# arkworks-rs/circom-compat

Hardware: AMD Instinct MI355X
Metric: Groth16 constraints/sec (BN254) (higher is better)
Workload: dtype int32x9 (29-bit limbs of 254-bit Montgomery integers); 1 GPU; synthetic squaring-chain R1CS, 2^22-2 constraints, BN254, full prove (witness map + 4 G1 MSM + 1 G2 MSM + finalize), trapdoor key minted on GPU; log2_domain=22, num_constraints=4194302, n_vars=4194304, parallelism=single-gpu

## Files before the change

circom_compat_amd/csrc/api.hip:

```cpp
#include "../../include/g16_amd.h"

#include <stddef.h>
#include <stdlib.h>

#include <algorithm>
#include <mutex>

#include "ctx.h"

using namespace g16;

static_assert(offsetof(g16::ProofSums, B1) == sizeof(g16::G1XYZZ29) && offsetof(g16::ProofSums, L) == 2 * sizeof(g16::G1XYZZ29),
              "ProofSums must keep A, B1, L adjacent (batched reduction writes them as an array)");
static_assert(G16_PARTIAL_BYTES == g16::FIN_PARTIAL_BYTES, "partial record size out of sync");

namespace {
std::mutex g_err_mu;
std::string g_create_error;
}


namespace {

g16_status fail(g16_ctx* ctx, g16_status code, const std::string& msg) {
  if (ctx) ctx->err = msg;
  else {
    std::lock_guard<std::mutex> g(g_err_mu);
    g_create_error = msg;
  }
  return code;
}

template <class Fn>
g16_status guarded(g16_ctx* ctx, Fn fn) {
  try {
    if (ctx) G16_HIP(hipSetDevice(ctx->device));
    return fn();
  } catch (const HipError& e) {
    return fail(ctx, G16_ERR_HIP, e.what());
  } catch (const std::bad_alloc&) {
    return fail(ctx, G16_ERR_INTERNAL, "host allocation failed");
  } catch (const std::exception& e) {
    const bool dom = std::string(e.what()).find("PolynomialDegreeTooLarge") != std::string::npos;
    return fail(ctx, dom ? G16_ERR_DOMAIN_TOO_LARGE : G16_ERR_INTERNAL, e.what());
  }
}

void shard(uint32_t len, int rank, int world, uint32_t* lo, uint32_t* hi) {
  *lo = (uint32_t)((uint64_t)len * rank / world);
  *hi = (uint32_t)((uint64_t)len * (rank + 1) / world);
}

int work1_batch(const MsmConfig& cw, uint32_t wr, bool sharded) {
  return (cw.nb() / wr < (1u << 18) || sharded) ? 3 : 2;
}

size_t msm_state_bytes(const MsmConfig& cw, const MsmConfig& ch, uint32_t lw, uint32_t l_cnt, uint32_t lh,
                       uint32_t wr, bool sharded, bool own_w, bool own_h, bool view_w) {
  size_t b = 0;
  if (view_w) b += MsmSort::view_bytes_for(lw, cw);
  if (own_w) b += (size_t)cw.Pn * ((size_t)lw * (64 * 2 + 128) + (size_t)l_cnt * 64);
  if (own_h) b += (size_t)ch.Pn * lh * 64;
  b += MsmSort::bytes_for(lw, cw) + MsmSort::bytes_for(lh, ch);
  const uint32_t nc_w = ceil_div(cw.B, msm_red_chunk(cw, 1, wr)) * cw.D;
  const uint32_t nc_h = ceil_div(ch.B, msm_red_chunk(ch)) * ch.D;
  const uint32_t slots_w = cw.nb() + cw.max_lanes(), slots_h = ch.nb() + ch.max_lanes();
  b += msm_work_bytes<Fq>(slots_w, nc_w, cw.D, work1_batch(cw, wr, sharded)) + msm_work_bytes<Fq2>(slots_w, nc_w, cw.D, 1) +
       msm_work_bytes<Fq>(slots_h, nc_h, ch.D, 1);
  return b;
}

void plan_msm_configs(const g16_options& o, uint32_t lw, uint32_t l_cnt, uint32_t lh, uint32_t wr, bool sharded,
                      bool own_w, bool own_h, bool view_w, MsmConfig* cw, MsmConfig* ch) {
  if (own_w) *cw = msm_make_config(lw ? lw : 1, o.window_bits, o.planes);
  if (own_h) *ch = msm_make_config(lh ? lh : 1, o.window_bits, o.planes);
  if (o.planes > 0) return;
  size_t fr = 0, tot = 0;
  if (hipMemGetInfo(&fr, &tot) != hipSuccess) return;
  const size_t margin = std::min(((size_t)2 << 30) + fr / 50, fr / 4);
  const size_t budget = fr - margin;
  if (msm_state_bytes(*cw, *ch, lw, l_cnt, lh, wr, sharded, own_w, own_h, view_w) <= budget) return;
  auto layouts = [&](const MsmConfig& full, uint32_t len, bool own) {
    std::vector<MsmConfig> v{full};
    for (int pn = full.Pn - 1; own && pn >= 1; --pn) {
      const MsmConfig c = msm_make_config(len ? len : 1, o.window_bits, pn);
      if (c.Pn != v.back().Pn) v.push_back(c);
    }
    return v;
  };
  const std::vector<MsmConfig> vw = layouts(*cw, lw, own_w), vh = layouts(*ch, lh, own_h);
  long best = -1;
  size_t best_bytes = 0;
  for (const MsmConfig& a : vw)
    for (const MsmConfig& b : vh) {
      const size_t need = msm_state_bytes(a, b, lw, l_cnt, lh, wr, sharded, own_w, own_h, view_w);
      if (need > budget) continue;
      const long score = 5L * a.D + b.D;
      if (best < 0 || score < best || (score == best && need > best_bytes)) {
        best = score;
        best_bytes = need;
        *cw = a;
        *ch = b;
      }
    }
  if (best < 0) {
    if (!own_w && !own_h)
      throw std::runtime_error("the sort and partial-sum state of this ctx does not fit the device memory that is free (" +
                               std::to_string(fr >> 20) + " MiB)");
    throw std::runtime_error("the proving key does not fit this device's memory even with one plane per point (" +
                             std::to_string(fr >> 20) + " MiB free)");
  }
}

inline bool sched_r5() {
  static const bool v = [] { const char* e = getenv("G16_SCHED_R5"); return e && atoi(e) != 0; }();
  return v;
}

void collect_times(g16_ctx* c) {
  if (c->timer.enabled) c->timer.collect(c->st_ms, c->st_cnt);
}

struct BucketChunk {
  uint32_t count;
  const Fr* w;
  size_t w_stride;
  int32_t *abc, *spmv;
  U256* h;
  ProofSums* sums;
  MsmSort *sort_w, *sort_h, *sort_b;
  MsmWork<Fq> *work1, *workH;
  MsmWork<Fq2>* work2;
  Fr* rs;
  const uint8_t* rs_host;
  FinScratch* scr;
  uint8_t *rec, *proj;
  uint32_t rec_stride;
  uint8_t *rec_host, *proj_host;
  const MsmSort& sort_for_b(const g16_ctx* c) const { return c->sparse_b ? *sort_b : *sort_w; }
};

BucketChunk own_chunk(g16_ctx* c, const Fr* w_dev) {
  return BucketChunk{1,           w_dev,       c->N,        c->wm.abc.p, c->wm.spmv.partial.p, c->h_canon.p, c->sums_dev.p,
                     &c->sort_w,  &c->sort_h,  &c->sort_b,  &c->work1,   &c->workH,            &c->work2,
                     c->rs_dev.p, c->pin_io,   c->fin_scr.p, c->out_dev.p, c->part_dev(), (uint32_t)G16_PROOF_BYTES,
                     c->pin_io + 64, c->pin_io + 64 + G16_PROOF_BYTES};
}

void accumulate_ab(g16_ctx* c, const BucketChunk& ch, hipStream_t s, StageTimer* tm, bool fixup = true) {
  if (c->ptsA.stride == 2) {
    msm_accumulate_pair<Fq>(*ch.sort_w, c->ptsA, c->ptsB1, *ch.work1, 0, s, tm, fixup);
  } else {
    msm_accumulate<Fq>(*ch.sort_w, c->ptsA, 0, *ch.work1, 0, s, tm, fixup);
    msm_accumulate<Fq>(*ch.sort_w, c->ptsB1, 0, *ch.work1, 1, s, tm, fixup);
  }
}
void fixup_ab(g16_ctx* c, const BucketChunk& ch, hipStream_t q) {
  StageTimer* tm = c->timer.enabled ? &c->timer : nullptr;
  if (c->ptsA.stride == 2) {
    msm_fixup_pair<Fq>(*ch.sort_w, c->ptsA, c->ptsB1, *ch.work1, 0, q, tm);
  } else {
    msm_fixup<Fq>(*ch.sort_w, c->ptsA, 0, *ch.work1, 0, q, tm);
    msm_fixup<Fq>(*ch.sort_w, c->ptsB1, 0, *ch.work1, 1, q, tm);
  }
}

void enqueue_witness_sort(g16_ctx* c, const BucketChunk& ch) {
  hipStream_t s = c->stream;
  StageTimer* tm = c->timer.enabled ? &c->timer : nullptr;
  int id = tm ? tm->begin(ST_MSM_SORT, s) : -1;
  ch.sort_w->run(ch.w + 1 + c->w_lo, c->w_hi - c->w_lo, true, s, ch.count, ch.w_stride);
  if (tm) tm->end(id, s);
  if (c->sparse_b) {
    hipStream_t v = c->overlap ? c->red : s;
    G16_HIP(hipEventRecord(c->ev_view, s));
    G16_HIP(hipStreamWaitEvent(v, c->ev_view, 0));
    id = tm ? tm->begin(ST_MSM_SORT, v) : -1;
    ch.sort_b->run_view(*ch.sort_w, c->keep_b, v);
    if (tm) tm->end(id, v);
    G16_HIP(hipEventRecord(c->ev_view, v));
  }
}
void wait_for_b_view(g16_ctx* c, hipStream_t s) {
  if (c->sparse_b) G16_HIP(hipStreamWaitEvent(s, c->ev_view, 0));
}

template <class Hook, class Hook2>
void enqueue_witness_msms(g16_ctx* c, const BucketChunk& ch, Hook after_ab, Hook2 after_b2, bool sorted = false) {
  hipStream_t s = c->stream;
  StageTimer* tm = c->timer.enabled ? &c->timer : nullptr;
  ProofSums* S = ch.sums;
  const size_t ps = sizeof(ProofSums);
  if (!sorted) enqueue_witness_sort(c, ch);
  const uint32_t nb_eff = ch.count * c->cfg_w.nb() / (c->shard_buckets ? (uint32_t)c->world : 1u);
  const bool small = nb_eff < (1u << 18);
  const uint32_t b2_limit = c->world > 1 ? (1u << 18) : (1u << 16);
  const bool b2_off = c->overlap && nb_eff < b2_limit;
  const bool sharded = c->world > 1 || c->dist_wm;
  const bool mid = (nb_eff >= (1u << 15) && small) || (sharded && nb_eff >= (1u << 15));
  if (mid && c->overlap && ch.work1->batch >= 3) {
    hipStream_t q = c->red;
    accumulate_ab(c, ch, s, tm, false);
    G16_HIP(hipEventRecord(c->ev_acc[0], s));
    G16_HIP(hipStreamWaitEvent(q, c->ev_acc[0], 0));
    fixup_ab(c, ch, q);
    msm_reduce<Fq>(*ch.sort_w, *ch.work1, 0, 2, &S->A, q, tm, true, ps);
    after_ab(q);
    wait_for_b_view(c, s);
    msm_accumulate<Fq2>(ch.sort_for_b(c), c->ptsB2, 0, *ch.work2, 0, s, tm);
    G16_HIP(hipEventRecord(c->ev_acc[1], s));
    G16_HIP(hipStreamWaitEvent(q, c->ev_acc[1], 0));
    msm_reduce<Fq2>(ch.sort_for_b(c), *ch.work2, 0, 1, &S->B2, q, tm, true, ps);
    const bool r5 = sched_r5();
    hipStream_t ql = r5 ? q : c->side;
    if (!r5) after_b2();
    msm_accumulate<Fq>(*ch.sort_w, c->ptsL, c->l_idx_min, *ch.work1, 2, s, tm, false);
    G16_HIP(hipEventRecord(c->ev_acc[2], s));
    G16_HIP(hipStreamWaitEvent(ql, c->ev_acc[2], 0));
    msm_fixup<Fq>(*ch.sort_w, c->ptsL, c->l_idx_min, *ch.work1, 2, ql, tm);
    msm_reduce<Fq>(*ch.sort_w, *ch.work1, 2, 1, &S->L, ql, tm, true, ps);
    if (r5) after_b2();
    G16_HIP(hipEventRecord(c->ev_b2, q));
    G16_HIP(hipStreamWaitEvent(c->side, c->ev_b2, 0));
    G16_HIP(hipEventRecord(c->ev_side, c->side));
    return;
  }
  if (small && ch.work1->batch >= 3) {
    accumulate_ab(c, ch, s, tm);
    msm_accumulate<Fq>(*ch.sort_w, c->ptsL, c->l_idx_min, *ch.work1, 2, s, tm);
    msm_reduce<Fq>(*ch.sort_w, *ch.work1, 0, 3, &S->A, s, tm, false, ps);
    after_ab(s);
  } else {
    accumulate_ab(c, ch, s, tm);
    msm_reduce<Fq>(*ch.sort_w, *ch.work1, 0, 2, &S->A, s, tm, false, ps);
    after_ab(s);
    msm_run<Fq>(*ch.sort_w, c->ptsL, c->l_idx_min, *ch.work1, &S->L, s, tm, ps);
  }
  wait_for_b_view(c, s);
  msm_accumulate<Fq2>(ch.sort_for_b(c), c->ptsB2, 0, *ch.work2, 0, s, tm);
  hipStream_t rs = b2_off ? c->red : s;
  G16_HIP(hipEventRecord(c->ev_b2, s));
  G16_HIP(hipStreamWaitEvent(rs, c->ev_b2, 0));
  msm_reduce<Fq2>(ch.sort_for_b(c), *ch.work2, 0, 1, &S->B2, rs, tm, false, ps);
  G16_HIP(hipEventRecord(c->ev_b2, rs));
  if (rs != c->red) G16_HIP(hipStreamWaitEvent(c->red, c->ev_b2, 0));
  after_b2();
  G16_HIP(hipEventRecord(c->ev_b2, c->red));
  G16_HIP(hipStreamWaitEvent(c->side, c->ev_b2, 0));
  G16_HIP(hipEventRecord(c->ev_side, c->side));
}

void enqueue_h_msm(g16_ctx* c, const BucketChunk& ch) {
  hipStream_t s = c->stream;
  StageTimer* tm = c->timer.enabled ? &c->timer : nullptr;
  G16_HIP(hipStreamWaitEvent(s, c->ev_h, 0));
  msm_run<Fq>(*ch.sort_h, c->ptsH, 0, *ch.workH, &ch.sums->H, s, tm, sizeof(ProofSums));
}

template <class Hook, class Hook2>
void run_msms(g16_ctx* c, const BucketChunk& ch, Hook after_ab, Hook2 after_b2) {
  hipStream_t s = c->stream, x = c->overlap ? c->aux : c->stream;
  StageTimer* tm = c->timer.enabled ? &c->timer : nullptr;
  const uint32_t nb_eff = ch.count * c->cfg_w.nb() / (c->shard_buckets ? (uint32_t)c->world : 1u);
  const bool sort_first = !sched_r5() && c->overlap && c->world == 1 && nb_eff >= (1u << 18) && c->n <= (1u << 24);
  if (sort_first) enqueue_witness_sort(c, ch);
  G16_HIP(hipEventRecord(c->ev_w, s));
  G16_HIP(hipStreamWaitEvent(x, c->ev_w, 0));
  int id = tm ? tm->begin(ST_WITNESS_MAP, x) : -1;
  c->wm.run_batch(ch.w, ch.w_stride, ch.count, ch.abc, ch.spmv, ch.h, nullptr, x);
  if (tm) tm->end(id, x);
  id = tm ? tm->begin(ST_MSM_SORT, x) : -1;
  ch.sort_h->run(ch.h + c->h_lo, c->h_hi - c->h_lo, false, x, ch.count, c->wm.n);
  if (tm) tm->end(id, x);
  G16_HIP(hipEventRecord(c->ev_h, x));
  enqueue_witness_msms(c, ch, after_ab, after_b2, sort_first);
  enqueue_h_msm(c, ch);
}

template <class Hook>
void run_msms(g16_ctx* c, const BucketChunk& ch, Hook after_ab) {
// ... 209 lines not shown

g16_status ctx_create_impl(const g16_key_desc* key, const g16_csr* a, const g16_csr* b,
                           uint32_t num_constraints, const g16_options* opt, g16_ctx* share_from,
                           g16_ctx** out, std::string* err) {
  auto bad = [&](g16_status code, const std::string& msg) {
    if (err) *err = msg;
    return code;
  };
  if (!key || !a || !b || !out) return bad(G16_ERR_INVALID, "null argument");
  *out = nullptr;
  g16_options o{};
  if (opt) o = *opt;
  if (o.world <= 0) o.world = 1;
  if (o.rank < 0 || o.rank >= o.world) return bad(G16_ERR_INVALID, "bad rank/world");
  if (o.shard < G16_SHARD_AUTO || o.shard > G16_SHARD_BUCKETS) return bad(G16_ERR_INVALID, "unknown shard mode");
  if ((uint64_t)key->n_vars < (uint64_t)key->n_public + 1)
    return bad(G16_ERR_INVALID, "n_vars < n_public+1");
  for (const g16_csr* mtx : {a, b}) {
    if (!mtx->row_ptr || (mtx->nnz && (!mtx->col || !mtx->coeff)))
      return bad(G16_ERR_INVALID, "matrix with null arrays");
    if (mtx->row_ptr[0] != 0 || mtx->row_ptr[num_constraints] != mtx->nnz)
      return bad(G16_ERR_INVALID, "matrix row_ptr does not span [0, nnz]");
    for (uint32_t i = 0; i < num_constraints; ++i)
      if (mtx->row_ptr[i] > mtx->row_ptr[i + 1])
        return bad(G16_ERR_INVALID, "matrix row_ptr is not monotone");
    for (uint64_t j = 0; j < mtx->nnz; ++j)
      if (mtx->col[j] >= key->n_vars)
        return bad(G16_ERR_INVALID, "matrix wire index >= n_vars");
  }
  int ndev = 0;
  if (hipGetDeviceCount(&ndev) != hipSuccess || ndev <= 0)
    return bad(G16_ERR_NO_DEVICE, "no HIP device visible: this library has no CPU fallback");
  if (o.device < 0 || o.device >= ndev) return bad(G16_ERR_INVALID, "bad device ordinal");
  if (share_from && (share_from->device != o.device || !share_from->has_key || share_from->multi ||
                     !(share_from->shard_buckets || (share_from->world == 1 && o.world == 1 && !share_from->dist_wm && o.dist_wm <= 0))))
    return bad(G16_ERR_INVALID, "planes can only be shared with a whole-key ctx on the same device");

  g16_ctx* c = new (std::nothrow) g16_ctx();
  if (!c) return bad(G16_ERR_INTERNAL, "host allocation failed");
  c->device = o.device;
  c->rank = o.rank;
  c->world = o.world;
  g16_status st = guarded(c, [&]() -> g16_status {
    G16_HIP(hipStreamCreateWithFlags(&c->stream, hipStreamNonBlocking));
    G16_HIP(hipStreamCreateWithFlags(&c->side, hipStreamNonBlocking));
    G16_HIP(hipStreamCreateWithFlags(&c->red, hipStreamNonBlocking));
    {
      int lo = 0, hi = 0;
      G16_HIP(hipDeviceGetStreamPriorityRange(&lo, &hi));
      (void)lo;
      G16_HIP(hipStreamCreateWithPriority(&c->aux, hipStreamNonBlocking, hi));
    }
    if (const char* e = getenv("G16_NO_OVERLAP")) c->overlap = !(e[0] == '1');
    G16_HIP(hipEventCreateWithFlags(&c->ev_w, hipEventDisableTiming));
    G16_HIP(hipEventCreateWithFlags(&c->ev_h, hipEventDisableTiming));
    G16_HIP(hipEventCreateWithFlags(&c->ev_start, hipEventDisableTiming));
    G16_HIP(hipEventCreateWithFlags(&c->ev_ab, hipEventDisableTiming));
    G16_HIP(hipEventCreateWithFlags(&c->ev_side, hipEventDisableTiming));
    G16_HIP(hipEventCreateWithFlags(&c->ev_b2, hipEventDisableTiming));
    for (auto& e : c->ev_acc) G16_HIP(hipEventCreateWithFlags(&e, hipEventDisableTiming));
    G16_HIP(hipEventCreateWithFlags(&c->ev_fixed, hipEventDisableTiming));
    G16_HIP(hipEventCreateWithFlags(&c->ev_view, hipEventDisableTiming));
    G16_HIP(hipEventCreateWithFlags(&c->ev_send, hipEventDisableTiming));
    G16_HIP(hipEventCreateWithFlags(&c->ev_part, hipEventDisableTiming));
    G16_HIP(hipEventCreateWithFlags(&c->ev_user, hipEventDisableTiming));
    hipStream_t s = c->stream;
    c->N = key->n_vars;
    c->p = key->n_public;
    c->num_inputs = c->p + 1;
    c->m = num_constraints;
    c->nnz_a = a->nnz;
    c->nnz_b = b->nnz;
    CsrHost A{a->row_ptr, a->col, (const Fr*)a->coeff, (size_t)a->nnz};
    CsrHost B{b->row_ptr, b->col, (const Fr*)b->coeff, (size_t)b->nnz};
    if (o.reduction != G16_REDUCTION_CIRCOM && o.reduction != G16_REDUCTION_LIBSNARK)
      throw std::runtime_error("unknown reduction");
    c->dist_wm = o.dist_wm > 0;
    if (c->dist_wm && o.reduction != G16_REDUCTION_CIRCOM)
      throw std::runtime_error("the distributed witness map implements CircomReduction only");
    if (c->dist_wm) {
      c->wd.init(A, B, c->m, c->num_inputs, c->rank, c->world);
      c->n = c->wd.n;
    } else {
      c->wm.init(A, B, c->m, c->num_inputs, o.reduction);
      c->n = c->wm.n;
    }
    if (key->domain_size != c->n)
      throw std::runtime_error("key domain_size does not match num_constraints + num_inputs");

    const uint32_t len_w = c->N - 1;
    c->has_key = key->a_query != nullptr;
    c->shard_buckets = c->world > 1 && c->has_key && o.shard == G16_SHARD_BUCKETS;
    c->share_from = (c->shard_buckets || c->world == 1) ? share_from : nullptr;
    if (c->share_from) ++c->share_from->borrowers;
    shard(len_w, c->rank, c->world, &c->w_lo, &c->w_hi);
    shard(c->n, c->rank, c->world, &c->h_lo, &c->h_hi);
    if (c->dist_wm) {
      c->h_lo = 0;
      c->h_hi = c->n / (uint32_t)c->world;
    }
    if (c->shard_buckets) {
      c->w_lo = 0;
      c->w_hi = len_w;
    }
    const uint32_t lw = c->w_hi - c->w_lo, lh = c->h_hi - c->h_lo;
    const uint32_t wr = c->shard_buckets ? (uint32_t)c->world : 1u;
// ... 966 lines not shown
```

circom_compat_amd/csrc/ctx.h:

```cpp
#pragma once
#include <atomic>
#include "../../include/g16_amd.h"

#include <memory>
#include <string>

#include "finalize.h"
#include "msm_table.h"
#include "msm.h"
#include "witness_map.h"
#include "wm_dist.h"

namespace g16 {
struct Multi;
}

struct g16_ctx {
  int device = 0, rank = 0, world = 1;
  uint32_t N = 0, p = 0, n = 0, m = 0, num_inputs = 0;
  bool has_key = false;
  bool overlap = true;
  hipStream_t stream = nullptr;
  hipStream_t side = nullptr;
  hipStream_t aux = nullptr;
  hipStream_t red = nullptr;
  hipEvent_t ev_start = nullptr, ev_ab = nullptr, ev_side = nullptr, ev_w = nullptr, ev_h = nullptr,
             ev_b2 = nullptr, ev_fixed = nullptr, ev_view = nullptr;
  hipEvent_t ev_acc[3] = {nullptr, nullptr, nullptr};
  hipEvent_t ev_send = nullptr;
  hipEvent_t ev_part = nullptr;
  hipEvent_t ev_user = nullptr;
  hipStream_t xstream = nullptr;
  bool have_xstream = false;
  void* nccl_comm = nullptr;
  int nccl_ranks = 0;
  hipStream_t xs_own = nullptr;
  g16::DevBuf<uint8_t> xsend, xrecv;
  std::string err;

  g16::WitnessMap wm;
  g16::WmDist wd;
  bool dist_wm = false;
  bool fixed_ready = false;
  uint64_t fixed_rs[8] = {0};
  bool shard_buckets = false;
  uint32_t w_lo = 0, w_hi = 0, h_lo = 0, h_hi = 0;
  uint32_t l_idx_min = 0;
  g16::MsmConfig cfg_w, cfg_h;
  g16::MsmSort sort_w, sort_h;
  g16::MsmSort sort_b;
  g16::DevBuf<uint32_t> keep_b_own;
  const uint32_t* keep_b = nullptr;
  bool sparse_b = false;
  uint32_t b_inf_points = 0;
  const g16::MsmSort& sort_for_b() const { return sparse_b ? sort_b : sort_w; }
  g16::MsmPoints<g16::Fq> ptsA, ptsB1, ptsL, ptsH;
  g16::MsmPoints<g16::Fq2> ptsB2;
  g16::MsmWork<g16::Fq> work1, workH;
  g16::MsmWork<g16::Fq2> work2;
  g16::TableSet tbl;

  g16::DevBuf<g16::Fr> w_dev, h_dev, rs_dev;
  g16::DevBuf<g16::U256> h_canon;
  g16::DevBuf<g16::KeyHeaderDev> key_dev;
  g16::DevBuf<g16::ProofSums> sums_dev;
  g16::DevBuf<g16::FinTables> fin_tab;
  g16::DevBuf<g16::FinScratch> fin_scr;
  g16::DevBuf<uint8_t> out_dev;
  void* pinned_w = nullptr;
  uint8_t* pin_io = nullptr;

  struct BatchWs {
    uint32_t cap = 0;
    g16::DevBuf<g16::Fr> w, rs;
// ... 58 lines not shown
```

circom_compat_amd/csrc/msm.h:

```cpp
#pragma once
#include <stdlib.h>
#include "common.h"
#include "ec29.h"

namespace g16 {

constexpr int MSM_ACC_THREADS = 128;
#ifdef G16_EMU
constexpr int MSM_ACC_BLOCKS = 48;
constexpr int MSM_ACC_BLOCKS_G2 = 32;
#else
constexpr int MSM_ACC_BLOCKS = 3072;
constexpr int MSM_ACC_BLOCKS_G2 = 2048;
#endif
constexpr int MSM_MIN_SEG = 8;
constexpr int MSM_SMALL_MULTI = 32;
constexpr int MSM_RED_CHUNK = 16;
constexpr uint32_t MSM_IDX_BITS_WIDE = 27, MSM_IDX_BITS_NARROW = 26;

struct MsmConfig {
  int c = 0;
  int W = 0;
  int Pn = 1;
  int D = 0;
// ... 92 lines not shown
  const Affine<F>* view = nullptr;
  uint32_t stride = 1, off = 0;
  const Affine<F>* data() const { return view ? view : pts.p; }
  void init(const Affine<F>* host_points, uint32_t count, const MsmConfig& cfg, hipStream_t stream);
  static void init_pair(MsmPoints& a, MsmPoints& b, const Affine<F>* host_a, const Affine<F>* host_b,
                        uint32_t count, const MsmConfig& cfg, hipStream_t stream);
  void init_from_device(const Affine<F>* dev_points, uint32_t count, const MsmConfig& cfg,
                        hipStream_t stream);
};

#ifdef G16_EMU
constexpr uint32_t MSM_FIX_CAP = 512;
#else
constexpr uint32_t MSM_FIX_CAP = 2048;
#endif
struct MsmFixList {
  uint32_t count;
  uint32_t overflow;
  uint32_t slot[MSM_FIX_CAP];
  uint32_t entry[MSM_FIX_CAP];
};

template <class F>
struct MsmWork {
  int batch = 1;
  uint32_t slots = 0, ncontrib = 0;
  int sets = 1;
  DevBuf<MsmAcc<F>> partial;
  DevBuf<MsmAcc<F>> contrib;
  DevBuf<MsmAcc<F>> bsum;
  DevBuf<MsmAcc<F>> wsum;
  DevBuf<MsmFixList> fix;
  void init(uint32_t n_slots, uint32_t n_contrib, int max_sets, int batch = 1);
};

template <class F>
inline size_t msm_work_bytes(uint32_t n_slots, uint32_t n_contrib, int max_sets, int batch) {
  return (size_t)batch * ((size_t)n_slots + n_contrib + (size_t)257 * max_sets) * sizeof(MsmAcc<F>) +
         (size_t)batch * sizeof(MsmFixList);
}

template <class F>
void msm_run(const MsmSort& s, const MsmPoints<F>& pts, uint32_t idx_min, MsmWork<F>& work,
             MsmAcc<F>* out_dev, hipStream_t stream, StageTimer* tm = nullptr, size_t out_stride = 0);
template <class F>
void msm_accumulate(const MsmSort& s, const MsmPoints<F>& pts, uint32_t idx_min, MsmWork<F>& work,
                    int slot, hipStream_t stream, StageTimer* tm = nullptr, bool fixup = true);
template <class F>
void msm_fixup(const MsmSort& s, const MsmPoints<F>& pts, uint32_t idx_min, MsmWork<F>& work, int slot,
               hipStream_t stream, StageTimer* tm = nullptr);
template <class F>
void msm_accumulate_pair(const MsmSort& s, const MsmPoints<F>& a, const MsmPoints<F>& b,
                         MsmWork<F>& work, int slot, hipStream_t stream, StageTimer* tm = nullptr,
                         bool fixup = true);
template <class F>
void msm_fixup_pair(const MsmSort& s, const MsmPoints<F>& a, const MsmPoints<F>& b, MsmWork<F>& work,
                    int slot, hipStream_t stream, StageTimer* tm = nullptr);
template <class F>
void msm_reduce(const MsmSort& s, MsmWork<F>& work, int first_slot, int nbatch, MsmAcc<F>* out_dev,
                hipStream_t stream, StageTimer* tm = nullptr, bool hidden = false, size_t out_stride = 0);
inline uint32_t msm_contrib_cap(const MsmConfig& cfg, uint32_t nproof_cap) {
  uint32_t m = 1;
  for (uint32_t z = 1; z <= nproof_cap; ++z)
    for (uint32_t nbatch = 1; nbatch <= 3; ++nbatch)
      for (int hidden = 0; hidden < 2; ++hidden) {
        const uint32_t rc = msm_red_chunk(cfg, nbatch * z, 1, hidden != 0);
        const uint32_t v = (uint32_t)(((uint64_t)cfg.B + rc - 1) / rc) * (uint32_t)cfg.D * z;
        if (v > m) m = v;
      }
  return m;
}



}
```

circom_compat_amd/csrc/msm_curve.inc.h:

```cpp
#pragma once
#include <stdlib.h>

#include "msm.h"

namespace g16 {

namespace {

constexpr int ACC_THREADS = MSM_ACC_THREADS;
constexpr uint32_t MSM_EXACT_BLOCKS = 256;

inline bool acc_fast() {
  static const bool v = [] { const char* e = getenv("G16_ACC_FAST"); return !e || atoi(e) != 0; }();
  return v;
}
template <class F>
constexpr bool acc_is_g1() { return sizeof(F) == sizeof(Fq); }
constexpr int COMB_THREADS = 64;
constexpr int SUM_THREADS = 128;

template <class F>
__global__ void __launch_bounds__(128) k_precompute_planes(Affine<F>* pts, uint32_t count, int Pn,
                                                           int shift_bits, uint32_t stride,
                                                           uint32_t off) {
  using LF = typename Lazy<F>::type;
  const uint32_t i = blockIdx.x * blockDim.x + threadIdx.x;
  if (i >= count) return;
  pts += off;
  const Aff29<LF> p0 = affine_from_mont256<F>(pts[(size_t)i * stride]);
  pts[(size_t)i * stride] = store_packed_affine<F>(p0);
  XYZZ29<LF> q = XYZZ29<LF>::from_affine(p0);
  for (int j = 1; j < Pn; ++j) {
    for (int s = 0; s < shift_bits; ++s) q.dbl_in_place();
    pts[((size_t)j * count + i) * stride] = store_packed_affine<F>(q.to_affine());
  }
}

__device__ __forceinline__ uint32_t bucket_of(const uint32_t* __restrict__ offset, uint32_t nb,
                                              uint32_t pos) {
  uint32_t lo = 0, hi = nb;
  while (hi - lo > 1) {
    const uint32_t mid = (lo + hi) >> 1;
    if (offset[mid] <= pos) lo = mid;
    else hi = mid;
  }
  return lo;
}

template <class F>
struct AccWay {
  using LF = typename Lazy<F>::type;
  uint32_t seg, pos, end, g, bend, bnext, en_next, en_next2;
  bool live;
  XYZZ29<LF> acc;
  Affine<F> raw_next;
};

__device__ uint32_t g_gather_mask = 0xffffffffu;

template <class F, int PS>
__device__ __forceinline__ void acc_fetch(const Affine<F>* __restrict__ pts, uint32_t npts,
                                          uint32_t idx_min, uint32_t idx_bits, uint32_t en,
                                          Affine<F>& raw) {
  const uint32_t idx = en & ((1u << idx_bits) - 1u);
  if (idx >= idx_min) {
    const uint32_t plane = (en & 0x7fffffffu) >> idx_bits;
#ifdef G16_DEBUG_GATHER
    raw = pts[((size_t)(plane & g_gather_mask) * npts + ((idx - idx_min) & g_gather_mask)) * PS];
#else
    raw = pts[((size_t)plane * npts + (idx - idx_min)) * PS];
#endif
  } else {
    raw = Affine<F>::infinity();
  }
}

template <class F, int PS>
__device__ __forceinline__ void acc_way_init(AccWay<F>& w, uint32_t seg, uint32_t S, uint32_t M,
                                             const Affine<F>* __restrict__ pts, uint32_t npts,
                                             uint32_t idx_min, uint32_t idx_bits,
                                             const uint32_t* __restrict__ entries,
                                             const uint32_t* __restrict__ offset, uint32_t nb) {
  w.seg = seg;
  w.pos = seg * S;
  w.live = w.pos < M;
  w.end = w.live ? (w.pos + S < M ? w.pos + S : M) : w.pos;
  w.acc = XYZZ29<typename Lazy<F>::type>::infinity();
  w.raw_next = Affine<F>::infinity();
  w.g = 0;
  w.bend = w.bnext = 0;
  w.en_next = w.en_next2 = 0;
  if (w.live) {
    w.g = bucket_of(offset, nb, w.pos);
    w.bend = offset[w.g + 1];
    w.bnext = offset[w.g + 2 < nb ? w.g + 2 : nb];
    w.en_next = entries[w.pos];
    w.en_next2 = w.pos + 1 < w.end ? entries[w.pos + 1] : 0u;
    acc_fetch<F, PS>(pts, npts, idx_min, idx_bits, w.en_next, w.raw_next);
  }
}

template <class F, int PS>
__device__ __forceinline__ Aff29<typename Lazy<F>::type> acc_way_prepare(
    AccWay<F>& w, bool* step, const Affine<F>* __restrict__ pts, uint32_t npts, uint32_t idx_min,
    uint32_t idx_bits, const uint32_t* __restrict__ entries, const uint32_t* __restrict__ offset,
    uint32_t nb, MsmAcc<F>* __restrict__ partial) {
  using LF = typename Lazy<F>::type;
  *step = w.live && w.pos < w.end;
  const uint32_t en = w.en_next;
  Aff29<LF> p = load_packed_affine<F>(w.raw_next);
  if (en >> 31) p.y = p.y.neg().carry();
  if (!*step) p.inf = true;
  if (*step && w.pos == w.bend) {
    partial[w.g + w.seg] = w.acc;
    w.acc = XYZZ29<LF>::infinity();
    ++w.g;
    w.bend = w.bnext;
    while (w.bend == w.pos) {
      ++w.g;
      w.bend = offset[w.g + 1];
    }
  }
  if (*step) w.bnext = offset[w.g + 2 < nb ? w.g + 2 : nb];
  w.en_next = w.en_next2;
  if (*step && w.pos + 2 < w.end) w.en_next2 = entries[w.pos + 2];
  if (*step && w.pos + 1 < w.end) acc_fetch<F, PS>(pts, npts, idx_min, idx_bits, w.en_next, w.raw_next);
  return p;
}

template <class F, bool FAST>
__device__ __forceinline__ void acc_way_commit(AccWay<F>& w, bool step,
                                               const XYZZ29<typename Lazy<F>::type>& res, bool special,
                                               const Aff29<typename Lazy<F>::type>& p, uint32_t en,
                                               uint32_t half, MsmFixList* fix) {
  if (FAST) {
    if (special) {
      const uint32_t k = atomicAdd(&fix->count, 1u);
      if (k < MSM_FIX_CAP) {
        fix->slot[k] = (w.g + w.seg) | (half << 31);
        fix->entry[k] = en;
      }
    } else {
      w.acc = res;
    }
  } else {
    if (special) w.acc.madd(p);
    else w.acc = res;
  }
  if (step) ++w.pos;
}

#ifdef G16_ACC_WAVES2
#define G16_ACC_ATTR __attribute__((amdgpu_waves_per_eu(2, 2)))
#else
#define G16_ACC_ATTR
#endif
template <class F, int PS, bool PAIR, bool FAST>
__global__ void __launch_bounds__(ACC_THREADS) G16_ACC_ATTR
    k_bucket_accumulate(const Affine<F>* __restrict__ pts, uint32_t npts, uint32_t idx_min,
                        uint32_t idx_bits, const uint32_t* __restrict__ entries,
                        const uint32_t* __restrict__ offset, uint32_t nb, uint32_t lanes,
                        MsmAcc<F>* __restrict__ partial, size_t slot_stride, MsmFixList* fix) {
  using LF = typename Lazy<F>::type;
  if (!FAST && fix && fix->overflow == 0) return;
  const uint32_t M = offset[nb];
  const uint32_t S = msm_seg_len(M, lanes);
  uint32_t nthreads = gridDim.x * blockDim.x, t0 = blockIdx.x * blockDim.x + threadIdx.x;
  uint32_t half = 0;
  if (PAIR) {
    half = threadIdx.x / (ACC_THREADS / 2);
    pts += half;
    partial += (size_t)half * slot_stride;
    nthreads /= 2;
    t0 = blockIdx.x * (ACC_THREADS / 2) + threadIdx.x % (ACC_THREADS / 2);
  }
  for (; t0 < lanes; t0 += nthreads) {
    AccWay<F> w;
    acc_way_init<F, PS>(w, t0, S, M, pts, npts, idx_min, idx_bits, entries, offset, nb);
    if (!w.live) break;
    for (uint32_t it = 0; it < S; ++it) {
      bool step, special;
      const uint32_t en = w.en_next;
      const Aff29<LF> p =
          acc_way_prepare<F, PS>(w, &step, pts, npts, idx_min, idx_bits, entries, offset, nb, partial);
      const XYZZ29<LF> r = XYZZ29<LF>::madd_select(w.acc, p, &special);
      acc_way_commit<F, FAST>(w, step, r, special, p, en, half, fix);
    }
    partial[w.g + w.seg] = w.acc;
  }
}

template <class F, int PS>
__global__ void __launch_bounds__(256)
    k_acc_fixup(const Affine<F>* __restrict__ pts, uint32_t npts, uint32_t idx_min, uint32_t idx_bits,
                MsmFixList* fix, MsmAcc<F>* partial, size_t slot_stride) {
  __shared__ uint32_t sl[MSM_FIX_CAP];
  __shared__ uint32_t done[MSM_FIX_CAP];
  __shared__ uint32_t left;
  const uint32_t n = fix->count;
  __syncthreads();
  if (threadIdx.x == 0) {
    fix->overflow = n > MSM_FIX_CAP ? 1u : 0u;
    fix->count = 0;
  }
  if (n == 0 || n > MSM_FIX_CAP) return;
  for (uint32_t i = threadIdx.x; i < n; i += blockDim.x) {
    sl[i] = fix->slot[i];
    done[i] = 0;
  }
  if (threadIdx.x == 0) left = n;
  __syncthreads();
  while (left != 0) {
    for (uint32_t i = threadIdx.x; i < n; i += blockDim.x) {
      if (done[i]) continue;
      bool first = true;
      for (uint32_t j = 0; j < i; ++j)
        if (done[j] != 1 && sl[j] == sl[i]) first = false;
      if (!first) continue;
      const uint32_t en = fix->entry[i], half = sl[i] >> 31, slot = sl[i] & 0x7fffffffu;
      Affine<F> raw;
      acc_fetch<F, PS>(pts + half, npts, idx_min, idx_bits, en, raw);
      Aff29<typename Lazy<F>::type> p = load_packed_affine<F>(raw);
      if (en >> 31) p.y = p.y.neg().carry();
      MsmAcc<F>* dst = partial + (size_t)half * slot_stride + slot;
      MsmAcc<F> a = *dst;
      a.madd(p);
      *dst = a;
      done[i] = 2;
    }
    __syncthreads();
    if (threadIdx.x == 0) {
      uint32_t l = 0;
      for (uint32_t i = 0; i < n; ++i) {
        if (done[i] == 2) done[i] = 1;
        if (!done[i]) ++l;
      }
      left = l;
    }
    __syncthreads();
  }
}
// ... 259 lines not shown
      MsmFixList* fix = work.fix.p + slot;
      if (P.stride == 2)
        G16_LAUNCH((k_bucket_accumulate<F, 2, false, true>), grid, ACC_THREADS, 0, stream, P.data() + P.off,
                   P.count, idx_min, cfg.idx_bits, en, of, nb, lanes, out, (size_t)0, fix);
      else
        G16_LAUNCH((k_bucket_accumulate<F, 1, false, true>), grid, ACC_THREADS, 0, stream, P.data(), P.count,
                   idx_min, cfg.idx_bits, en, of, nb, lanes, out, (size_t)0, fix);
      if (tm) tm->end(id, stream);
      if (fixup) msm_fixup<F>(s, P, idx_min, work, slot, stream, tm);
      return;
    }
  }
  if (P.stride == 2)
    G16_LAUNCH((k_bucket_accumulate<F, 2, false, false>), grid, ACC_THREADS, 0, stream, P.data() + P.off,
               P.count, idx_min, cfg.idx_bits, en, of, nb, lanes, out, (size_t)0, (MsmFixList*)nullptr);
  else
    G16_LAUNCH((k_bucket_accumulate<F, 1, false, false>), grid, ACC_THREADS, 0, stream, P.data(), P.count,
               idx_min, cfg.idx_bits, en, of, nb, lanes, out, (size_t)0, (MsmFixList*)nullptr);
  if (tm) tm->end(id, stream);
}

template <class F>
void msm_fixup(const MsmSort& s, const MsmPoints<F>& P, uint32_t idx_min, MsmWork<F>& work, int slot,
               hipStream_t stream, StageTimer* tm) {
  if constexpr (!acc_is_g1<F>()) {
    return;
  } else {
  if (!acc_fast()) return;
  const int tid = tm ? tm->begin(ST_MSM_FIXUP, stream) : -1;
  const MsmConfig& cfg = s.cfg;
  const uint32_t nb = s.nbt();
  const uint32_t lanes = s.lanes_of(sizeof(F) != sizeof(Fq));
  const uint32_t grid = lanes / ACC_THREADS;
  MsmAcc<F>* out = work.partial.p + (size_t)slot * work.slots;
  const uint32_t* en = (const uint32_t*)s.entries.p;
  const uint32_t* of = (const uint32_t*)s.offset.p;
  MsmFixList* fix = work.fix.p + slot;
  const uint32_t grid_x = grid < MSM_EXACT_BLOCKS ? grid : MSM_EXACT_BLOCKS;
  if (P.stride == 2) {
    G16_LAUNCH((k_acc_fixup<F, 2>), 1, 256, 0, stream, P.data() + P.off, P.count, idx_min, cfg.idx_bits, fix, out, (size_t)0);
    G16_LAUNCH((k_bucket_accumulate<F, 2, false, false>), grid_x, ACC_THREADS, 0, stream, P.data() + P.off,
               P.count, idx_min, cfg.idx_bits, en, of, nb, lanes, out, (size_t)0, fix);
  } else {
    G16_LAUNCH((k_acc_fixup<F, 1>), 1, 256, 0, stream, P.data(), P.count, idx_min, cfg.idx_bits, fix, out, (size_t)0);
    G16_LAUNCH((k_bucket_accumulate<F, 1, false, false>), grid_x, ACC_THREADS, 0, stream, P.data(), P.count,
               idx_min, cfg.idx_bits, en, of, nb, lanes, out, (size_t)0, fix);
  }
  if (tm) tm->end(tid, stream);
  }
}

template <class F>
void msm_accumulate_pair(const MsmSort& s, const MsmPoints<F>& A, const MsmPoints<F>& B,
                         MsmWork<F>& work, int slot, hipStream_t stream, StageTimer* tm, bool fixup) {
  const MsmConfig& cfg = s.cfg;
  const uint32_t nb = s.nbt();
  const int acc_stage = ST_MSM_ACC_G1_PAIR;
  if (slot < 0 || slot + 2 > work.batch) throw std::runtime_error("msm_accumulate_pair: bad workspace slot");
  if (A.stride != 2 || B.stride != 2 || A.data() != B.data() || A.off != 0 || B.off != 1 ||
      A.count != B.count)
    throw std::runtime_error("msm_accumulate_pair: the queries are not an interleaved pair");
  const uint32_t grid = cfg.lanes / (ACC_THREADS / 2);
  int id = tm ? tm->begin(acc_stage, stream) : -1;
  const uint32_t* en = (const uint32_t*)s.entries.p;
  const uint32_t* of = (const uint32_t*)s.offset.p;
  MsmAcc<F>* out = work.partial.p + (size_t)slot * work.slots;
  if constexpr (sizeof(F) == sizeof(Fq)) {
    if (acc_fast()) {
      G16_LAUNCH((k_bucket_accumulate<F, 2, true, true>), grid, ACC_THREADS, 0, stream, A.data(), A.count, 0u,
                 cfg.idx_bits, en, of, nb, cfg.lanes, out, (size_t)work.slots, work.fix.p + slot);
      if (tm) tm->end(id, stream);
      if (fixup) msm_fixup_pair<F>(s, A, B, work, slot, stream, tm);
      return;
    }
  }
  G16_LAUNCH((k_bucket_accumulate<F, 2, true, false>), grid, ACC_THREADS, 0, stream, A.data(), A.count, 0u,
             cfg.idx_bits, en, of, nb, cfg.lanes, out, (size_t)work.slots, (MsmFixList*)nullptr);
  if (tm) tm->end(id, stream);
}

template <class F>
void msm_fixup_pair(const MsmSort& s, const MsmPoints<F>& A, const MsmPoints<F>& B, MsmWork<F>& work,
                    int slot, hipStream_t stream, StageTimer* tm) {
  (void)B;
  if constexpr (sizeof(F) == sizeof(Fq)) {
    if (!acc_fast()) return;
    const int tid = tm ? tm->begin(ST_MSM_FIXUP, stream) : -1;
    const MsmConfig& cfg = s.cfg;
    const uint32_t nb = s.nbt();
    const uint32_t grid = cfg.lanes / (ACC_THREADS / 2);
    MsmAcc<F>* out = work.partial.p + (size_t)slot * work.slots;
    MsmFixList* fix = work.fix.p + slot;
    const uint32_t grid_x = grid < MSM_EXACT_BLOCKS ? grid : MSM_EXACT_BLOCKS;
    G16_LAUNCH((k_acc_fixup<F, 2>), 1, 256, 0, stream, A.data(), A.count, 0u, cfg.idx_bits, fix, out, (size_t)work.slots);
    G16_LAUNCH((k_bucket_accumulate<F, 2, true, false>), grid_x, ACC_THREADS, 0, stream, A.data(), A.count, 0u,
               cfg.idx_bits, (const uint32_t*)s.entries.p, (const uint32_t*)s.offset.p, nb, cfg.lanes, out,
               (size_t)work.slots, fix);
    if (tm) tm->end(tid, stream);
  }
}

template <class F>
void msm_reduce(const MsmSort& s, MsmWork<F>& work, int first_slot, int nbatch, MsmAcc<F>* out_dev,
                hipStream_t stream, StageTimer* tm, bool hidden, size_t out_stride) {
  const MsmConfig& cfg = s.cfg;
  const uint32_t nb = s.nbt();
  const uint32_t sets = (uint32_t)cfg.D * s.nproof;
  if (first_slot < 0 || nbatch < 1 || first_slot + nbatch > work.batch)
    throw std::runtime_error("msm_reduce: bad workspace slots");
  MsmAcc<F>* partial = work.partial.p + (size_t)first_slot * work.slots;
  int id = tm ? tm->begin(ST_MSM_REDUCE, stream) : -1;
  const bool g2 = sizeof(F) != sizeof(Fq);
  const uint32_t lanes = s.lanes_of(g2);
  G16_LAUNCH((k_combine_large<F>), dim3(1024, nbatch), COMB_THREADS, COMB_THREADS * sizeof(MsmAcc<F>),
             stream, s.large_list(g2), s.large_meta(g2),
             (const uint32_t*)s.offset.p, nb, lanes, partial, (size_t)work.slots);
  const uint32_t* rng = s.range_dev();
  const uint32_t red_chunk = msm_red_chunk(cfg, (uint32_t)nbatch * s.nproof, (uint32_t)s.world, hidden);
  const uint32_t cps = ceil_div(cfg.B, red_chunk);
  const uint32_t nchunks = cps * sets;
  if (nchunks > work.ncontrib) throw std::runtime_error("msm_reduce: contribution buffer too small");
  if ((int)sets > work.sets) throw std::runtime_error("msm_reduce: more bucket sets than the workspace holds");
  MsmAcc<F>* contrib = work.contrib.p + (size_t)first_slot * work.ncontrib;
  MsmAcc<F>* bsum = work.bsum.p + (size_t)first_slot * 256 * work.sets;
  MsmAcc<F>* wsum = work.wsum.p + (size_t)first_slot * work.sets;
  G16_LAUNCH((k_bucket_reduce<F>), dim3(ceil_div(nchunks, 64), nbatch), 64, 0, stream,
             (const MsmAcc<F>*)partial, (const uint32_t*)s.offset.p, nb, lanes, cfg.B, red_chunk,
             cps, nchunks, contrib, (size_t)work.slots, rng);
  uint32_t nblk = ceil_div(cps / (uint32_t)s.world, SUM_THREADS * 2);
  if (nblk > 256) nblk = 256;
  if (nblk < 1) nblk = 1;
  G16_LAUNCH((k_set_sum<F>), dim3(sets * nblk, nbatch), SUM_THREADS,
             SUM_THREADS * sizeof(MsmAcc<F>), stream, (const MsmAcc<F>*)contrib, cps, nblk,
             bsum, (size_t)nchunks, (size_t)256 * work.sets, rng, red_chunk);
  G16_LAUNCH((k_set_sum<F>), dim3(sets, nbatch), SUM_THREADS,
             SUM_THREADS * sizeof(MsmAcc<F>), stream, (const MsmAcc<F>*)bsum, nblk, 1u,
             wsum, (size_t)256 * work.sets, (size_t)work.sets, (const uint32_t*)nullptr, 1u);
  G16_LAUNCH((k_horner<F>), dim3(nbatch, s.nproof), 64, 0, stream, (const MsmAcc<F>*)wsum, work.sets, cfg.D,
             cfg.c, out_dev, out_stride);
  if (tm) tm->end(id, stream);
}

template <class F>
void msm_run(const MsmSort& s, const MsmPoints<F>& P, uint32_t idx_min, MsmWork<F>& work,
             MsmAcc<F>* out_dev, hipStream_t stream, StageTimer* tm, size_t out_stride) {
  msm_accumulate<F>(s, P, idx_min, work, 0, stream, tm);
  msm_reduce<F>(s, work, 0, 1, out_dev, stream, tm, false, out_stride);
}

}
// ... 1 lines not shown
```

circom_compat_amd/csrc/msm_g1.hip:

```cpp
#include "msm_curve.inc.h"
namespace g16 {
template struct MsmPoints<Fq>;
template struct MsmWork<Fq>;
template void msm_run<Fq>(const MsmSort&, const MsmPoints<Fq>&, uint32_t, MsmWork<Fq>&, MsmAcc<Fq>*,
                          hipStream_t, StageTimer*, size_t);
template void msm_accumulate<Fq>(const MsmSort&, const MsmPoints<Fq>&, uint32_t, MsmWork<Fq>&, int,
                                 hipStream_t, StageTimer*, bool);
template void msm_fixup<Fq>(const MsmSort&, const MsmPoints<Fq>&, uint32_t, MsmWork<Fq>&, int, hipStream_t, StageTimer*);
template void msm_accumulate_pair<Fq>(const MsmSort&, const MsmPoints<Fq>&, const MsmPoints<Fq>&,
                                      MsmWork<Fq>&, int, hipStream_t, StageTimer*, bool);
template void msm_fixup_pair<Fq>(const MsmSort&, const MsmPoints<Fq>&, const MsmPoints<Fq>&, MsmWork<Fq>&, int,
                                 hipStream_t, StageTimer*);
template void msm_reduce<Fq>(const MsmSort&, MsmWork<Fq>&, int, int, MsmAcc<Fq>*, hipStream_t,
                             StageTimer*, bool, size_t);
}
```

Measured before the change: 115.1 million constraints/s.

## Share pair-record fetch across waves via LDS and batch large A/B1/L reductions

```diff
diff --git a/circom_compat_amd/csrc/api.hip b/circom_compat_amd/csrc/api.hip
--- a/circom_compat_amd/csrc/api.hip
+++ b/circom_compat_amd/csrc/api.hip
@@ -52,7 +52,8 @@
 }
 
 int work1_batch(const MsmConfig& cw, uint32_t wr, bool sharded) {
-  return (cw.nb() / wr < (1u << 18) || sharded) ? 3 : 2;
+  (void)cw; (void)wr; (void)sharded;
+  return 3;
 }
 
 size_t msm_state_bytes(const MsmConfig& cw, const MsmConfig& ch, uint32_t lw, uint32_t l_cnt, uint32_t lh,
@@ -149,7 +150,7 @@
 
 void accumulate_ab(g16_ctx* c, const BucketChunk& ch, hipStream_t s, StageTimer* tm, bool fixup = true) {
   if (c->ptsA.stride == 2) {
-    msm_accumulate_pair<Fq>(*ch.sort_w, c->ptsA, c->ptsB1, *ch.work1, 0, s, tm, fixup);
+    msm_accumulate_pair<Fq>(*ch.sort_w, c->ptsA, c->ptsB1, *ch.work1, 0, s, tm, fixup, c->pair_fetch_twice);
   } else {
     msm_accumulate<Fq>(*ch.sort_w, c->ptsA, 0, *ch.work1, 0, s, tm, fixup);
     msm_accumulate<Fq>(*ch.sort_w, c->ptsB1, 0, *ch.work1, 1, s, tm, fixup);
@@ -158,7 +159,7 @@
 void fixup_ab(g16_ctx* c, const BucketChunk& ch, hipStream_t q) {
   StageTimer* tm = c->timer.enabled ? &c->timer : nullptr;
   if (c->ptsA.stride == 2) {
-    msm_fixup_pair<Fq>(*ch.sort_w, c->ptsA, c->ptsB1, *ch.work1, 0, q, tm);
+    msm_fixup_pair<Fq>(*ch.sort_w, c->ptsA, c->ptsB1, *ch.work1, 0, q, tm, c->pair_fetch_twice);
   } else {
     msm_fixup<Fq>(*ch.sort_w, c->ptsA, 0, *ch.work1, 0, q, tm);
     msm_fixup<Fq>(*ch.sort_w, c->ptsB1, 0, *ch.work1, 1, q, tm);
@@ -197,7 +198,8 @@
   const uint32_t b2_limit = c->world > 1 ? (1u << 18) : (1u << 16);
   const bool b2_off = c->overlap && nb_eff < b2_limit;
   const bool sharded = c->world > 1 || c->dist_wm;
-  const bool mid = (nb_eff >= (1u << 15) && small) || (sharded && nb_eff >= (1u << 15));
+  const bool batched_large = !sharded && !c->red_split && ch.work1->batch >= 3 && nb_eff >= c->red_batch_min;
+  const bool mid = !batched_large && ((nb_eff >= (1u << 15) && small) || (sharded && nb_eff >= (1u << 15)));
   if (mid && c->overlap && ch.work1->batch >= 3) {
     hipStream_t q = c->red;
     accumulate_ab(c, ch, s, tm, false);
@@ -225,7 +227,7 @@
     G16_HIP(hipEventRecord(c->ev_side, c->side));
     return;
   }
-  if (small && ch.work1->batch >= 3) {
+  if ((small || batched_large) && ch.work1->batch >= 3) {
     accumulate_ab(c, ch, s, tm);
     msm_accumulate<Fq>(*ch.sort_w, c->ptsL, c->l_idx_min, *ch.work1, 2, s, tm);
     msm_reduce<Fq>(*ch.sort_w, *ch.work1, 0, 3, &S->A, s, tm, false, ps);
@@ -541,6 +543,9 @@
       G16_HIP(hipStreamCreateWithPriority(&c->aux, hipStreamNonBlocking, hi));
     }
     if (const char* e = getenv("G16_NO_OVERLAP")) c->overlap = !(e[0] == '1');
+    if (const char* e = getenv("G16_PAIR_FETCH_TWICE")) c->pair_fetch_twice = atoi(e) != 0;
+    if (const char* e = getenv("G16_RED_SPLIT")) c->red_split = atoi(e) != 0;
+    if (const char* e = getenv("G16_RED_BATCH_MIN_BUCKETS")) c->red_batch_min = (uint32_t)strtoul(e, nullptr, 0);
     G16_HIP(hipEventCreateWithFlags(&c->ev_w, hipEventDisableTiming));
     G16_HIP(hipEventCreateWithFlags(&c->ev_h, hipEventDisableTiming));
     G16_HIP(hipEventCreateWithFlags(&c->ev_start, hipEventDisableTiming));
diff --git a/circom_compat_amd/csrc/ctx.h b/circom_compat_amd/csrc/ctx.h
--- a/circom_compat_amd/csrc/ctx.h
+++ b/circom_compat_amd/csrc/ctx.h
@@ -20,6 +20,9 @@
   uint32_t N = 0, p = 0, n = 0, m = 0, num_inputs = 0;
   bool has_key = false;
   bool overlap = true;
+  bool pair_fetch_twice = false;
+  bool red_split = false;
+  uint32_t red_batch_min = 1u << 18;
   hipStream_t stream = nullptr;
   hipStream_t side = nullptr;
   hipStream_t aux = nullptr;
diff --git a/circom_compat_amd/csrc/msm.h b/circom_compat_amd/csrc/msm.h
--- a/circom_compat_amd/csrc/msm.h
+++ b/circom_compat_amd/csrc/msm.h
@@ -168,10 +168,10 @@
 template <class F>
 void msm_accumulate_pair(const MsmSort& s, const MsmPoints<F>& a, const MsmPoints<F>& b,
                          MsmWork<F>& work, int slot, hipStream_t stream, StageTimer* tm = nullptr,
-                         bool fixup = true);
+                         bool fixup = true, bool fetch_twice = false);
 template <class F>
 void msm_fixup_pair(const MsmSort& s, const MsmPoints<F>& a, const MsmPoints<F>& b, MsmWork<F>& work,
-                    int slot, hipStream_t stream, StageTimer* tm = nullptr);
+                    int slot, hipStream_t stream, StageTimer* tm = nullptr, bool fetch_twice = false);
 template <class F>
 void msm_reduce(const MsmSort& s, MsmWork<F>& work, int first_slot, int nbatch, MsmAcc<F>* out_dev,
                 hipStream_t stream, StageTimer* tm = nullptr, bool hidden = false, size_t out_stride = 0);
diff --git a/circom_compat_amd/csrc/msm_curve.inc.h b/circom_compat_amd/csrc/msm_curve.inc.h
--- a/circom_compat_amd/csrc/msm_curve.inc.h
+++ b/circom_compat_amd/csrc/msm_curve.inc.h
@@ -75,12 +75,63 @@
   }
 }
 
-template <class F, int PS>
+struct alignas(16) RecPiece {
+  uint32_t x, y, z, w;
+};
+constexpr int ACC_REC_PIECES = 4;
+constexpr int ACC_REC_BUF = ACC_REC_PIECES * 64;
+
+template <class F>
+__device__ __forceinline__ const Affine<F>* acc_record_of(const Affine<F>* __restrict__ pts, uint32_t npts,
+                                                          uint32_t idx_min, uint32_t idx_bits, uint32_t en) {
+  const uint32_t idx = en & ((1u << idx_bits) - 1u);
+  const uint32_t plane = (en & 0x7fffffffu) >> idx_bits;
+#ifdef G16_DEBUG_GATHER
+  return pts + ((size_t)(plane & g_gather_mask) * npts + ((idx - idx_min) & g_gather_mask)) * 2;
+#else
+  return pts + ((size_t)plane * npts + (idx - idx_min)) * 2;
+#endif
+}
+
+template <class F>
+__device__ __forceinline__ void acc_fetch_record(const Affine<F>* __restrict__ pts, uint32_t npts,
+                                                 uint32_t idx_min, uint32_t idx_bits, uint32_t en,
+                                                 Affine<F>& raw, RecPiece* buf) {
+  static_assert(sizeof(Affine<F>) == ACC_REC_PIECES * sizeof(RecPiece), "half record = four 16-byte pieces");
+  if ((en & ((1u << idx_bits) - 1u)) >= idx_min) {
+    const RecPiece* src = reinterpret_cast<const RecPiece*>(acc_record_of<F>(pts, npts, idx_min, idx_bits, en) + 1);
+#ifdef G16_EMU
+    for (int k = 0; k < ACC_REC_PIECES; ++k) buf[k * 64 + (threadIdx.x & 63)] = src[k];
+#else
+    for (int k = 0; k < ACC_REC_PIECES; ++k)
+      __builtin_amdgcn_global_load_lds((const __attribute__((address_space(1))) void*)(src + k),
+                                       (__attribute__((address_space(3))) void*)(buf + k * 64), 16, 0, 0);
+#endif
+  }
+  acc_fetch<F, 2>(pts, npts, idx_min, idx_bits, en, raw);
+}
+
+template <class F>
+__device__ __forceinline__ Affine<F> acc_take_record(uint32_t idx_min, uint32_t idx_bits, uint32_t en,
+                                                     const RecPiece* buf) {
+  const uint32_t lane = threadIdx.x & 63;
+  const RecPiece a = buf[lane], b = buf[64 + lane], c = buf[128 + lane], d = buf[192 + lane];
+  Affine<F> raw;
+  raw.x.v[0] = a.x; raw.x.v[1] = a.y; raw.x.v[2] = a.z; raw.x.v[3] = a.w;
+  raw.x.v[4] = b.x; raw.x.v[5] = b.y; raw.x.v[6] = b.z; raw.x.v[7] = b.w;
+  raw.y.v[0] = c.x; raw.y.v[1] = c.y; raw.y.v[2] = c.z; raw.y.v[3] = c.w;
+  raw.y.v[4] = d.x; raw.y.v[5] = d.y; raw.y.v[6] = d.z; raw.y.v[7] = d.w;
+  if ((en & ((1u << idx_bits) - 1u)) < idx_min) raw = Affine<F>::infinity();
+  return raw;
+}
+
+template <class F, int PS, bool SHARE = false>
 __device__ __forceinline__ void acc_way_init(AccWay<F>& w, uint32_t seg, uint32_t S, uint32_t M,
                                              const Affine<F>* __restrict__ pts, uint32_t npts,
                                              uint32_t idx_min, uint32_t idx_bits,
                                              const uint32_t* __restrict__ entries,
-                                             const uint32_t* __restrict__ offset, uint32_t nb) {
+                                             const uint32_t* __restrict__ offset, uint32_t nb,
+                                             uint32_t half = 0, RecPiece* rec_buf = nullptr) {
   w.seg = seg;
   w.pos = seg * S;
   w.live = w.pos < M;
@@ -96,19 +147,32 @@
     w.bnext = offset[w.g + 2 < nb ? w.g + 2 : nb];
     w.en_next = entries[w.pos];
     w.en_next2 = w.pos + 1 < w.end ? entries[w.pos + 1] : 0u;
-    acc_fetch<F, PS>(pts, npts, idx_min, idx_bits, w.en_next, w.raw_next);
-  }
-}
-
-template <class F, int PS>
+    if constexpr (SHARE) {
+      if (half == 0) acc_fetch_record<F>(pts, npts, idx_min, idx_bits, w.en_next, w.raw_next, rec_buf);
+    } else {
+      acc_fetch<F, PS>(pts, npts, idx_min, idx_bits, w.en_next, w.raw_next);
+    }
+  }
+}
+
+template <class F, int PS, bool SHARE = false>
 __device__ __forceinline__ Aff29<typename Lazy<F>::type> acc_way_prepare(
     AccWay<F>& w, bool* step, const Affine<F>* __restrict__ pts, uint32_t npts, uint32_t idx_min,
     uint32_t idx_bits, const uint32_t* __restrict__ entries, const uint32_t* __restrict__ offset,
-    uint32_t nb, MsmAcc<F>* __restrict__ partial) {
+    uint32_t nb, MsmAcc<F>* __restrict__ partial, uint32_t half = 0, RecPiece* rec_sh = nullptr,
+    uint32_t par = 0) {
   using LF = typename Lazy<F>::type;
   *step = w.live && w.pos < w.end;
   const uint32_t en = w.en_next;
-  Aff29<LF> p = load_packed_affine<F>(w.raw_next);
+  Affine<F> raw = w.raw_next;
+  if constexpr (SHARE) {
+#ifndef G16_EMU
+    asm volatile("s_waitcnt vmcnt(0)" ::: "memory");
+#endif
+    __syncthreads();
+    if (half == 1) raw = acc_take_record<F>(idx_min, idx_bits, en, rec_sh + par * ACC_REC_BUF);
+  }
+  Aff29<LF> p = load_packed_affine<F>(raw);
   if (en >> 31) p.y = p.y.neg().carry();
   if (!*step) p.inf = true;
   if (*step && w.pos == w.bend) {
@@ -124,7 +188,14 @@
   if (*step) w.bnext = offset[w.g + 2 < nb ? w.g + 2 : nb];
   w.en_next = w.en_next2;
   if (*step && w.pos + 2 < w.end) w.en_next2 = entries[w.pos + 2];
-  if (*step && w.pos + 1 < w.end) acc_fetch<F, PS>(pts, npts, idx_min, idx_bits, w.en_next, w.raw_next);
+  if (*step && w.pos + 1 < w.end) {
+    if constexpr (SHARE) {
+      if (half == 0)
+        acc_fetch_record<F>(pts, npts, idx_min, idx_bits, w.en_next, w.raw_next, rec_sh + (par ^ 1u) * ACC_REC_BUF);
+    } else {
+      acc_fetch<F, PS>(pts, npts, idx_min, idx_bits, w.en_next, w.raw_next);
+    }
+  }
   return p;
 }
 
@@ -155,7 +226,7 @@
 #else
 #define G16_ACC_ATTR
 #endif
-template <class F, int PS, bool PAIR, bool FAST>
+template <class F, int PS, bool PAIR, bool FAST, bool SHARE = false>
 __global__ void __launch_bounds__(ACC_THREADS) G16_ACC_ATTR
     k_bucket_accumulate(const Affine<F>* __restrict__ pts, uint32_t npts, uint32_t idx_min,
                         uint32_t idx_bits, const uint32_t* __restrict__ entries,
@@ -166,27 +237,35 @@
   const uint32_t M = offset[nb];
   const uint32_t S = msm_seg_len(M, lanes);
   uint32_t nthreads = gridDim.x * blockDim.x, t0 = blockIdx.x * blockDim.x + threadIdx.x;
-  uint32_t half = 0;
+  static_assert(!SHARE || (PAIR && PS == 2 && ACC_THREADS == 128), "SHARE: the two waves of a pair workgroup");
+  __shared__ RecPiece rec_sh[SHARE ? 2 * ACC_REC_BUF : 1];
+  uint32_t half = 0, par = 0;
   if (PAIR) {
     half = threadIdx.x / (ACC_THREADS / 2);
-    pts += half;
+    if (!SHARE) pts += half;
     partial += (size_t)half * slot_stride;
     nthreads /= 2;
     t0 = blockIdx.x * (ACC_THREADS / 2) + threadIdx.x % (ACC_THREADS / 2);
   }
   for (; t0 < lanes; t0 += nthreads) {
     AccWay<F> w;
-    acc_way_init<F, PS>(w, t0, S, M, pts, npts, idx_min, idx_bits, entries, offset, nb);
-    if (!w.live) break;
+    acc_way_init<F, PS, SHARE>(w, t0, S, M, pts, npts, idx_min, idx_bits, entries, offset, nb, half,
+                               rec_sh + par * ACC_REC_BUF);
+    if (SHARE) {
+      if ((uint64_t)(t0 - threadIdx.x % 64) * S >= M) break;
+    } else {
+      if (!w.live) break;
+    }
     for (uint32_t it = 0; it < S; ++it) {
       bool step, special;
       const uint32_t en = w.en_next;
-      const Aff29<LF> p =
-          acc_way_prepare<F, PS>(w, &step, pts, npts, idx_min, idx_bits, entries, offset, nb, partial);
+      const Aff29<LF> p = acc_way_prepare<F, PS, SHARE>(w, &step, pts, npts, idx_min, idx_bits, entries, offset,
+                                                        nb, partial, half, rec_sh, par);
+      if (SHARE) par ^= 1u;
       const XYZZ29<LF> r = XYZZ29<LF>::madd_select(w.acc, p, &special);
       acc_way_commit<F, FAST>(w, step, r, special, p, en, half, fix);
     }
-    partial[w.g + w.seg] = w.acc;
+    if (!SHARE || w.live) partial[w.g + w.seg] = w.acc;
   }
 }
 
@@ -552,7 +631,8 @@
 
 template <class F>
 void msm_accumulate_pair(const MsmSort& s, const MsmPoints<F>& A, const MsmPoints<F>& B,
-                         MsmWork<F>& work, int slot, hipStream_t stream, StageTimer* tm, bool fixup) {
+                         MsmWork<F>& work, int slot, hipStream_t stream, StageTimer* tm, bool fixup,
+                         bool fetch_twice) {
   const MsmConfig& cfg = s.cfg;
   const uint32_t nb = s.nbt();
   const int acc_stage = ST_MSM_ACC_G1_PAIR;
@@ -567,21 +647,29 @@
   MsmAcc<F>* out = work.partial.p + (size_t)slot * work.slots;
   if constexpr (sizeof(F) == sizeof(Fq)) {
     if (acc_fast()) {
-      G16_LAUNCH((k_bucket_accumulate<F, 2, true, true>), grid, ACC_THREADS, 0, stream, A.data(), A.count, 0u,
-                 cfg.idx_bits, en, of, nb, cfg.lanes, out, (size_t)work.slots, work.fix.p + slot);
+      if (fetch_twice)
+        G16_LAUNCH((k_bucket_accumulate<F, 2, true, true, false>), grid, ACC_THREADS, 0, stream, A.data(), A.count, 0u,
+                   cfg.idx_bits, en, of, nb, cfg.lanes, out, (size_t)work.slots, work.fix.p + slot);
+      else
+        G16_LAUNCH((k_bucket_accumulate<F, 2, true, true, true>), grid, ACC_THREADS, 0, stream, A.data(), A.count, 0u,
+                   cfg.idx_bits, en, of, nb, cfg.lanes, out, (size_t)work.slots, work.fix.p + slot);
       if (tm) tm->end(id, stream);
-      if (fixup) msm_fixup_pair<F>(s, A, B, work, slot, stream, tm);
+      if (fixup) msm_fixup_pair<F>(s, A, B, work, slot, stream, tm, fetch_twice);
       return;
     }
   }
-  G16_LAUNCH((k_bucket_accumulate<F, 2, true, false>), grid, ACC_THREADS, 0, stream, A.data(), A.count, 0u,
-             cfg.idx_bits, en, of, nb, cfg.lanes, out, (size_t)work.slots, (MsmFixList*)nullptr);
+  if (fetch_twice)
+    G16_LAUNCH((k_bucket_accumulate<F, 2, true, false, false>), grid, ACC_THREADS, 0, stream, A.data(), A.count, 0u,
+               cfg.idx_bits, en, of, nb, cfg.lanes, out, (size_t)work.slots, (MsmFixList*)nullptr);
+  else
+    G16_LAUNCH((k_bucket_accumulate<F, 2, true, false, true>), grid, ACC_THREADS, 0, stream, A.data(), A.count, 0u,
+               cfg.idx_bits, en, of, nb, cfg.lanes, out, (size_t)work.slots, (MsmFixList*)nullptr);
   if (tm) tm->end(id, stream);
 }
 
 template <class F>
 void msm_fixup_pair(const MsmSort& s, const MsmPoints<F>& A, const MsmPoints<F>& B, MsmWork<F>& work,
-                    int slot, hipStream_t stream, StageTimer* tm) {
+                    int slot, hipStream_t stream, StageTimer* tm, bool fetch_twice) {
   (void)B;
   if constexpr (sizeof(F) == sizeof(Fq)) {
     if (!acc_fast()) return;
@@ -593,9 +681,14 @@
     MsmFixList* fix = work.fix.p + slot;
     const uint32_t grid_x = grid < MSM_EXACT_BLOCKS ? grid : MSM_EXACT_BLOCKS;
     G16_LAUNCH((k_acc_fixup<F, 2>), 1, 256, 0, stream, A.data(), A.count, 0u, cfg.idx_bits, fix, out, (size_t)work.slots);
-    G16_LAUNCH((k_bucket_accumulate<F, 2, true, false>), grid_x, ACC_THREADS, 0, stream, A.data(), A.count, 0u,
-               cfg.idx_bits, (const uint32_t*)s.entries.p, (const uint32_t*)s.offset.p, nb, cfg.lanes, out,
-               (size_t)work.slots, fix);
+    if (fetch_twice)
+      G16_LAUNCH((k_bucket_accumulate<F, 2, true, false, false>), grid_x, ACC_THREADS, 0, stream, A.data(), A.count, 0u,
+                 cfg.idx_bits, (const uint32_t*)s.entries.p, (const uint32_t*)s.offset.p, nb, cfg.lanes, out,
+                 (size_t)work.slots, fix);
+    else
+      G16_LAUNCH((k_bucket_accumulate<F, 2, true, false, true>), grid_x, ACC_THREADS, 0, stream, A.data(), A.count, 0u,
+                 cfg.idx_bits, (const uint32_t*)s.entries.p, (const uint32_t*)s.offset.p, nb, cfg.lanes, out,
+                 (size_t)work.slots, fix);
     if (tm) tm->end(tid, stream);
   }
 }
diff --git a/circom_compat_amd/csrc/msm_g1.hip b/circom_compat_amd/csrc/msm_g1.hip
--- a/circom_compat_amd/csrc/msm_g1.hip
+++ b/circom_compat_amd/csrc/msm_g1.hip
@@ -8,9 +8,9 @@
                                  hipStream_t, StageTimer*, bool);
 template void msm_fixup<Fq>(const MsmSort&, const MsmPoints<Fq>&, uint32_t, MsmWork<Fq>&, int, hipStream_t, StageTimer*);
 template void msm_accumulate_pair<Fq>(const MsmSort&, const MsmPoints<Fq>&, const MsmPoints<Fq>&,
-                                      MsmWork<Fq>&, int, hipStream_t, StageTimer*, bool);
+                                      MsmWork<Fq>&, int, hipStream_t, StageTimer*, bool, bool);
 template void msm_fixup_pair<Fq>(const MsmSort&, const MsmPoints<Fq>&, const MsmPoints<Fq>&, MsmWork<Fq>&, int,
-                                 hipStream_t, StageTimer*);
+                                 hipStream_t, StageTimer*, bool);
 template void msm_reduce<Fq>(const MsmSort&, MsmWork<Fq>&, int, int, MsmAcc<Fq>*, hipStream_t,
                              StageTimer*, bool, size_t);
 }
```

After: 113.3 million constraints/s. 0.985x the previous value.
